# Mouafak-Khaled/Flow-Q-Learning

Hardware: AMD Instinct MI355X
Metric: FQL grad-steps/sec (whole node) over 16-α population, cube-single-v0 (higher is better)
Workload: dtype f32

## Files before the change

flow-q-learning_amd/csrc/kernels.h:

```cpp
#pragma once
#include <hip/hip_runtime.h>
#include <stdint.h>

namespace fq {

struct TRef {
    float* p;
    long long ss;
    long long sy;
};

inline TRef tref(float* p, long long ss, long long sy = 0) { return TRef{p, ss, sy}; }

enum GemmLayout { LAYOUT_FWD = 0, LAYOUT_DX = 1, LAYOUT_DW = 2 };
enum GemmEpi { EPI_STORE = 0, EPI_BIAS = 1, EPI_BIAS_GELU2 = 2, EPI_BIAS_GELU = 3, EPI_ADAM = 4 };

struct GemmArgs {
    TRef A, B, C, C2, bias;
    int M, N, K;
    int lda, ldb, ldc;
    int ny, nz;
    const int* slots;
    unsigned long long* probe;
};
// ... 217 lines not shown
    int nz;
    const int* slots;
};
void launch_input_grad(const InGradArgs& a, hipStream_t s);

struct SampleArgs {
    const float *obs, *act, *rew, *mask, *nobs;
    long long n_rows;
    const float* inj_batch;
    const float* inj_noise;
    const uint64_t* seeds;
    const int* count;
    int step_add;
    unsigned stream_salt;
    int B, D, A;
    TRef os_in;
    TRef bc_in;
    TRef cr_in;
    TRef tg_in;
    TRef eu_in;
    TRef act_t, x0_t, rew_t, mask_t;
    int nz;
    const int* slots;
};
void launch_sample(const SampleArgs& a, hipStream_t s);

struct LossArgs {
    TRef q, qt, rew, mask;
    TRef vpred, act, x0, amet;
    TRef apiraw, aflow, da;
    TRef dq;
    TRef dv;
    TRef dout_os;
    TRef g_cb4, g_bcb4, g_osb4;
    TRef info;
    const float* alpha;
    int B, A, E, da_n;
    int q_min, normq;
    float discount;
    int nz;
    const int* slots;
};
void launch_loss_critic(const LossArgs& a, hipStream_t s);
void launch_loss_bc(const LossArgs& a, hipStream_t s);
void launch_loss_actor(const LossArgs& a, hipStream_t s);

void launch_adam(const AdamArgs& a, hipStream_t s);

struct FinalArgs {
    const float* stats;
    const int* chunk_leaf;
    const int* leaf_first;
    int n_total_chunks, n_leaves;
// ... 52 lines not shown
```

flow-q-learning_amd/csrc/kernels.hip:

```cpp
#include "kernels.h"

#include <hip/hip_runtime.h>
#include <math.h>

#include <type_traits>

#if defined(__HIP_DEVICE_COMPILE__) && !defined(__gfx950__)
#error "fqlpop kernels target gfx950 (MI355X) only: the s_waitcnt immediates use the gfx9 encoding"
#endif


namespace fq {

typedef float f32x16 __attribute__((ext_vector_type(16)));
typedef float f32x4 __attribute__((ext_vector_type(4)));

#define DEV __device__ __forceinline__

DEV float* at(TRef t, int slot, int y = 0) {
    return t.p + (long long)slot * t.ss + (long long)y * t.sy;
}

constexpr float kSqrt2OverPi = 0.7978845608028654f;

// ... 2931 lines not shown
        obs = pb + (long long)b * D;
        actp = pb + (long long)B * D + (long long)b * A;
        rew = pb[(long long)B * (D + A) + b];
        mask = pb[(long long)B * (D + A + 1) + b];
        nobs = pb + (long long)B * (D + A + 2) + (long long)b * D;
    } else {
        const long long idx = (long long)(((unsigned long long)c0[0] * (unsigned long long)a.n_rows) >> 32);
        actp = a.act + idx * A;
        obs = a.obs + idx * D;
        nobs = a.nobs + idx * D;
        rew = a.rew[idx];
        mask = a.mask[idx];
    }
    const float* pn = a.inj_noise ? a.inj_noise + z * (long long)B * (4 * A + 1) : nullptr;
    const float t = pn ? pn[(long long)B * 2 * A + b] : u01(c0[1]);
    auto put = [&](int k, float o, float n) {
        os[k * B3 + b] = n;
        os[k * B3 + B + b] = o;
        os[k * B3 + 2 * B + b] = o;
        bc[k * B2 + b] = o;
        bc[k * B2 + B + b] = o;
        cr[k * B2 + b] = o;
        cr[k * B2 + B + b] = o;
        tg[(long long)k * B + b] = n;
        eu[(long long)k * B + b] = o;
    };
    constexpr int KQ = 8;
    float ov[KQ], nv0[KQ];
#pragma unroll
    for (int q = 0; q < KQ; ++q) {
        const int k = min(p + SP * q, D - 1);
        ov[q] = obs[k];
        nv0[q] = nobs[k];
    }
#pragma unroll
    for (int q = 0; q < KQ; ++q)
        if (p + SP * q < D) put(p + SP * q, ov[q], nv0[q]);
    for (int k = p + SP * KQ; k < D; k += SP) put(k, obs[k], nobs[k]);
    if (p < A) {
        const float av = actp[p];
        cr[(D + p) * B2 + b] = av;
        at(a.act_t, slot)[(long long)p * B + b] = av;
    }
    for (int q = p; 2 * q < 4 * A; q += SP) {
        float nv[2];
        if (pn) {
            for (int h = 0; h < 2; ++h) {
                const int i = 2 * q + h, cat = i / A, j = i % A;
                const long long o = cat == 0 ? (long long)b * A + j
                                  : cat == 1 ? (long long)B * A + b * A + j
                                  : cat == 2 ? (long long)B * (2 * A + 1) + b * A + j
                                             : (long long)B * (3 * A + 1) + b * A + j;
                nv[h] = i < 4 * A ? pn[o] : 0.f;
            }
        } else {
            uint32_t c[4] = {(uint32_t)b, step, a.stream_salt, 1u + (uint32_t)q};
            philox4x32_10(c, (uint32_t)seed, (uint32_t)(seed >> 32));
            const float r = sqrtf(-2.0f * logf(u01_open_closed(c[0])));
            float sv, cv;
            sincosf(6.283185307179586f * u01(c[1]), &sv, &cv);
            nv[0] = r * cv;
            nv[1] = r * sv;
        }
        for (int h = 0; h < 2; ++h) {
            const int i = 2 * q + h;
            if (i >= 4 * A) break;
            const int cat = i / A, j = i % A;
            const long long r = D + j;
            const float v = nv[h];
            if (cat == 0) {
                os[r * B3 + b] = v;
            } else if (cat == 1) {
                at(a.x0_t, slot)[(long long)j * B + b] = v;
                bc[r * B2 + b] = (1.0f - t) * v + t * actp[j];
            } else if (cat == 2) {
                os[r * B3 + B + b] = v;
                bc[r * B2 + B + b] = v;
            } else {
                os[r * B3 + 2 * B + b] = v;
            }
        }
// ... 39 lines not shown
            qs += qv;
            qmx = fmaxf(qmx, qv);
            qmn = fminf(qmn, qv);
            const float g = 2.0f * d * invEB;
            dq[e * a.dq.sy + b] = g;
            if (e < 4) sdq[e] += g;
            qp += q[e * a.q.sy + B + b];
        }
        qp /= (float)E;
        qpi_s += qp;
        qpi_abs += fabsf(qp);
    }
    const float* am = at(a.amet, slot);
    const float* ac = at(a.act, slot);
    float smse = 0.f;
    for (int i = threadIdx.x; i < A * B; i += 256) {
        const float d = am[i] - ac[i];
        smse += d * d;
    }
    float rv[11] = {sq, qs, qmx, qmn, qpi_s, qpi_abs, smse, sdq[0], sdq[1], sdq[2], sdq[3]};
    block_reduce_n<11>(rv, {0, 0, 1, 2, 0, 0, 0, 0, 0, 0, 0}, red);
    sq = rv[0];
    qs = rv[1];
    qmx = rv[2];
    qmn = rv[3];
    qpi_s = rv[4];
    qpi_abs = rv[5];
    smse = rv[6];
    if (threadIdx.x == 0)
        for (int e = 0; e < E && e < 4; ++e) at(a.g_cb4, slot, e)[0] = rv[7 + e];
    const float qmean_pi = qpi_s / (float)B;
    const float lam = a.normq ? 1.0f / (qpi_abs / (float)B) : 1.0f;
    const float gpi = -lam * invEB;
    for (int b = threadIdx.x; b < B; b += 256)
        for (int e = 0; e < E; ++e) dq[e * a.dq.sy + B + b] = gpi;
    if (threadIdx.x == 0) {
        float* info = at(a.info, slot);
        info[0] = sq * invEB;
        info[1] = qs * invEB;
        info[2] = qmx;
        info[3] = qmn;
        info[7] = -lam * qmean_pi;
        info[8] = qmean_pi;
        info[9] = smse / (float)(A * B);
    }
}

__global__ __launch_bounds__(256) void loss_bc_kernel(const LossArgs a) {
    const int z = blockIdx.x, slot = a.slots[z];
    const int B = a.B, A = a.A;
    __shared__ float red[9 * 8];
    const float* vp = at(a.vpred, slot);
    const float* ac = at(a.act, slot);
    const float* x0 = at(a.x0, slot);
    float* dv = at(a.dv, slot);
    const float sc = 2.0f / (float)(A * B);
    float s = 0.f;
    float sdb[8];
#pragma unroll
// ... 406 lines not shown
```

flow-q-learning_amd/csrc/runtime.cpp:

```cpp
#include <hip/hip_runtime.h>

#include <algorithm>
#include <cmath>
#include <cstdio>
#include <cstdlib>
#include <cstring>
#include <functional>
#include <map>
#include <set>
#include <memory>
#include <string>
#include <vector>

#include "../../include/fqlpop.h"
#include "kernels.h"

using namespace fq;

namespace {

thread_local std::string g_err;

struct FqErr {
    int code;
// ... 23 lines not shown

struct EngineOptions {
    int euler_fused = 1;
    int stream_fwd = 1;
    int stream_bwd = 1;
    int fused_adam = 1;
    int serial = 0;
    int dw_tile_critic = 10, dw_tile_actor = 10;
    int adam_nt = 3;
    int split = 1;
    int small_sched = 1;
    int split_blocks = 256;
    int split_sites = 0;
    int hw_queues = 4;
    int em_seq_sweep = 1;
};
EngineOptions g_engine_opts;

constexpr int kStepBranches = 4;
int step_streams(const EngineOptions& eo) {
    return (eo.serial || eo.hw_queues < kStepBranches) ? 1 : kStepBranches;
}

struct EngineOptionRef {
    const char* name;
    int EngineOptions::*field;
    int lo, hi;
};
const EngineOptionRef kEngineOptions[] = {
    {"euler_fused", &EngineOptions::euler_fused, 0, 1}, {"stream_fwd", &EngineOptions::stream_fwd, 0, 1},
    {"stream_bwd", &EngineOptions::stream_bwd, 0, 1},   {"fused_adam", &EngineOptions::fused_adam, 0, 1},
    {"serial", &EngineOptions::serial, 0, 1},
    {"dw_tile_critic", &EngineOptions::dw_tile_critic, 0, 10},
    {"dw_tile_actor", &EngineOptions::dw_tile_actor, 0, 10},
    {"adam_nt", &EngineOptions::adam_nt, 0, 3},
    {"split", &EngineOptions::split, 0, 8},
    {"small_sched", &EngineOptions::small_sched, 0, 1},
    {"hw_queues", &EngineOptions::hw_queues, 1, 1024},
    {"split_sites", &EngineOptions::split_sites, 0, (1 << 24) - 1},
    {"split_blocks", &EngineOptions::split_blocks, 64, 1024},
    {"em_seq_sweep", &EngineOptions::em_seq_sweep, 0, 1},
};

void philox_host(uint32_t c[4], uint32_t k0, uint32_t k1) {
    for (int r = 0; r < 10; ++r) {
        const uint64_t p0 = (uint64_t)0xD2511F53u * c[0], p1 = (uint64_t)0xCD9E8D57u * c[2];
        const uint32_t hi0 = (uint32_t)(p0 >> 32), lo0 = (uint32_t)p0;
        const uint32_t hi1 = (uint32_t)(p1 >> 32), lo1 = (uint32_t)p1;
        const uint32_t n0 = hi1 ^ c[1] ^ k0, n2 = hi0 ^ c[3] ^ k1;
        c[0] = n0; c[1] = lo1; c[2] = n2; c[3] = lo0;
        k0 += 0x9E3779B9u;
        k1 += 0xBB67AE85u;
    }
}

uint64_t sample_key(uint64_t seed, float alpha) {
// ... 142 lines not shown
    long long phase_blocks = 0;
    unsigned long long* ephase_host = nullptr;
    unsigned long long* ephase_dev = nullptr;
    long long ephase_blocks = 0;
    int probe_pairs = 0;
    long long probe_blocks = 0;
    long long probe_nb[2] = {0, 0};
    hipEvent_t probe_done[2] = {nullptr, nullptr};
    hipStream_t probe_stream = nullptr;
    bool probe_pending[2] = {false, false};
    double probe_total_ms = 0.0;
    long long probe_launches = 0;
    long long probe_blocks_seen = 0, probe_blocks_expected = 0;
    double clock_check_event_us = 0.0, clock_check_stamp_us = 0.0;
    std::map<long long, Graphs> graphs;

    float* alloc(long long per_slot) {
        float* p = nullptr;
        HIPCHK(hipMalloc(&p, sizeof(float) * std::max<long long>(1, per_slot * n)));
        HIPCHK(hipMemset(p, 0, sizeof(float) * std::max<long long>(1, per_slot * n)));
        allocs.push_back(p);
        return p;
    }
};

namespace {

void build_leaves(fqlpop* h) {
    struct NetRef { const char* name; int id; const NetLayout* lay; };
    const NetRef order[4] = {{"actor_bc_flow", 2, &h->bc}, {"actor_onestep_flow", 3, &h->os},
// ... 158 lines not shown
    mirror_params(h, slot, h->sM);
    HIPCHK(hipStreamSynchronize(h->sM));
    h->wt_dirty = true;
}

const NetLayout* phase_net(const fqlpop* h) {
    const char* v = diag_env("FQLPOP_PHASE_NET");
    if (v != nullptr && std::strcmp(v, "bc") == 0) return &h->bc;
    if (v != nullptr && std::strcmp(v, "os") == 0) return &h->os;
    return &h->critic;
}

struct Ctx {
    fqlpop* h;
    int nz;
};

TRef pref(fqlpop* h, float* arena, const NetLayout& N, long long off) {
    return tref(arena + N.off + off, h->P, N.ens_size);
}

hipEvent_t next_event(fqlpop* h) {
    if (h->ev_next >= (int)h->ev_pool.size()) throw FqErr{FQLPOP_E_STATE, "event pool exhausted"};
    return h->ev_pool[h->ev_next++];
}

struct TileChoice {
    int tile, variant;
};
TileChoice pick_gemm(int layout, int M, int N, int nyz) {
    const long long t64 = (long long)((M + 63) / 64) * (N / 64) * nyz;
    if (layout == LAYOUT_FWD) {
        if (M % 64 != 0) return {0, 0};
        if (t64 <= 512) return {0, 5};
        if (N % 128 == 0 && N < 768) return {2, 4};
        return {0, 4};
    }
    if (M < 64) return {0, 0};
    if (N % 128 != 0) return {0, 0};
    return {t64 >= 2048 ? 3 : 2, 0};
}

void gemm(int layout, int epi, const GemmArgs& g, hipStream_t s) {
    const TileChoice t = pick_gemm(layout, g.M, g.N, g.ny * g.nz);
    launch_gemm_variant(layout, epi, t.tile, t.variant, g, s);
}

constexpr long long kSmallSchedTiles = 256;
enum { SITE_BCF = 0, SITE_EULER = 1, SITE_OSF = 2, SITE_TGT = 3, SITE_CRF = 4, SITE_CRB = 5, SITE_OSB = 6, SITE_CRB2 = 7,
       SITE_N = 8 };
constexpr long long kSplitMaxClusters = 128;
constexpr long long kSplitMaxClustersSide = 64;
constexpr long long split_cap(int site) {
    return (site == SITE_BCF || site == SITE_TGT || site == SITE_CRF || site == SITE_OSB) ? kSplitMaxClustersSide
                                                                                        : kSplitMaxClusters;
}
constexpr long long kSplitMaxBlocks = 256;

int split_factor_opts(const EngineOptions& o, bool split_ok, int site, long long clusters, bool min4,
// ... 7 lines not shown
    }
    if (!split_ok || opt == 0 || clusters > split_cap(site)) return 1;
    for (int F = std::max(opt >= 2 ? opt : 8, min4 ? 4 : 2); F >= 2; F /= 2) {
        if (min4 && F < 4) break;
        if (clusters * F <= max_blocks) return F;
    }
    return 1;
}
int split_factor(const fqlpop* h, int site, long long clusters, bool min4, long long max_blocks = kSplitMaxBlocks) {
    return split_factor_opts(h->opt, h->split_ok, site, clusters, min4, max_blocks);
}

struct SplitShape {
    int H, L, A, B, E, K0bc, K0os, K0cr;
    bool critic_ln, stream_fwd, stream_bwd, fused_adam, euler_fused, multi_stream;
};
void split_plan(const EngineOptions& o, const SplitShape& d, int nz, int F[SITE_N], bool* small) {
    const bool ok = d.stream_fwd && o.split != 0;
    const int B = d.B, B2 = 2 * B, B3 = 3 * B, T = B / 16;
    auto fwd = [&](int site, int K0, int nout, int M, long long clusters, bool min4) {
        F[site] = d.stream_fwd && split_fwd_supported(d.H, d.L, K0, nout, M)
                      ? split_factor_opts(o, ok, site, clusters, min4, o.split_blocks) : 1;
    };
    fwd(SITE_EULER, d.K0bc, d.A, B, (long long)T * nz, true);
    if (!d.euler_fused) F[SITE_EULER] = 1;
    *small = o.small_sched && d.multi_stream && d.stream_fwd && d.stream_bwd && d.fused_adam &&
             (long long)T * nz <= kSmallSchedTiles;
    fwd(SITE_BCF, d.K0bc, d.A, B2, (long long)(B2 / 16) * nz, false);
    fwd(SITE_OSF, d.K0os, d.A, B3, (long long)(B3 / 16) * nz, false);
    fwd(SITE_TGT, d.K0cr, 1, B, (long long)T * d.E * nz, false);
    fwd(SITE_CRF, d.K0cr, 1, B2, (long long)(B2 / 16) * d.E * nz, false);
    auto bwd = [&](int site, int nout, int M, int Mg, long long clusters, bool min4) {
        F[site] = d.stream_bwd && split_bwd_supported(d.H, d.L, nout, M, Mg)
                      ? split_factor_opts(o, ok, site, clusters, min4, kSplitMaxBlocks) : 1;
    };
    if (*small) {
        bwd(SITE_CRB, 1, B, 0, (long long)T * d.E * nz, d.critic_ln);
        bwd(SITE_CRB2, 1, B, B, (long long)T * d.E * nz, d.critic_ln);
    } else {
        bwd(SITE_CRB, 1, B2, B, (long long)(B2 / 16) * d.E * nz, d.critic_ln);
        F[SITE_CRB2] = 1;
    }
    bwd(SITE_OSB, d.A, B, B, (long long)T * nz, false);
}
SplitShape split_shape(const fqlpop* h) {
    return SplitShape{h->H, h->L, h->A, h->B, h->E, h->bc.in_dim, h->os.in_dim, h->critic.in_dim, h->critic.ln,
                      h->stream_fwd, h->stream_bwd, h->fused_adam, h->euler_fused, h->sX != h->sM};
}
void check_plan(const fqlpop* h, int site, int nz, int F) {
    int plan[SITE_N];
    bool small = false;
    split_plan(h->opt, split_shape(h), nz, plan, &small);
    ARGCHK(plan[site] == F, "split launch differs from the split plan");
}

SplitSync split_prep(fqlpop* h, int site, long long clusters, hipStream_t) {
    fqlpop::SplitSite& st = h->split_site[site];
    ARGCHK(clusters <= st.clusters, "split launch larger than its site");
    return SplitSync{st.xch, st.cnt, st.gen, h->split_err};
}

int bwd_split(const fqlpop* h, int site, const NetLayout& N, int M, int Mg, int nz) {
    if (&N == &h->bc || !split_bwd_supported(N.H, N.L, N.out_dim, M, Mg)) return 1;
    return split_factor(h, site, (long long)(M / 16) * N.E * nz, N.ln, kSplitMaxBlocks);
}

void fwd_hidden(const Ctx& c, hipStream_t s, const NetLayout& N, TRef X, int ldx, int M,
                const std::vector<float*>& U, const std::vector<float*>& G, long long act_sy,
                const std::vector<float*>* MU, const std::vector<float*>* RS, long long st_sy,
                bool store_u, bool euler = false) {
    fqlpop* h = c.h;
    for (int l = 0; l < N.L; ++l) {
        GemmArgs g{};
        g.A = pref(h, h->params, N, N.W[l]);
        g.B = l == 0 ? X : tref(G[l - 1], (long long)N.H * ldx * N.E, act_sy);
        if (N.ln) {
            g.C = tref(U[l], (long long)N.H * ldx * N.E, act_sy);
        } else {
            g.C = tref(store_u ? U[l] : G[l], (long long)N.H * ldx * N.E, act_sy);
            g.C2 = tref(G[l], (long long)N.H * ldx * N.E, act_sy);
        }
        g.bias = pref(h, h->params, N, N.b[l]);
        g.M = N.H; g.N = M; g.K = N.kdim(l);
        g.lda = N.H; g.ldb = ldx; g.ldc = ldx;
        g.ny = N.E; g.nz = c.nz; g.slots = h->slots;
        const int epi = N.ln ? EPI_BIAS : (store_u ? EPI_BIAS_GELU2 : EPI_BIAS_GELU);
        if (euler && l >= 1 && epi == EPI_BIAS_GELU && g.M % 64 == 0 && g.N % 64 == 0) {
            if (h->probe_set >= 0 && h->probe_idx < h->probe_pairs)
                g.probe = h->probe_slots + 2 * h->probe_blocks * ((long long)h->probe_set * h->probe_pairs + h->probe_idx++);
            launch_gemm_euler_hidden(g, s);
        } else {
            gemm(LAYOUT_FWD, epi, g, s);
        }
        if (N.ln) {
            LnArgs a{};
            a.u = tref(U[l], (long long)N.H * ldx * N.E, act_sy);
            a.h = tref(G[l], (long long)N.H * ldx * N.E, act_sy);
            a.mu = tref((*MU)[l], (long long)ldx * N.E, st_sy);
            a.rstd = tref((*RS)[l], (long long)ldx * N.E, st_sy);
            a.gamma = pref(h, h->params, N, N.gam[l]);
            a.beta = pref(h, h->params, N, N.bet[l]);
            a.H = N.H; a.M = M; a.ld = ldx; a.ny = N.E; a.nz = c.nz; a.slots = h->slots;
            launch_ln_gelu_fwd(a, s);
        }
    }
}

// ... 114 lines not shown
    a.L = N.L; a.M = M; a.Mg = Mg; a.nout = N.out_dim;
    a.ny = N.E; a.nz = c.nz; a.slots = h->slots;
    if (ig) {
        ARGCHK(ig->off == Mg && ig->M == M - Mg, "input-grad columns must follow the grad columns");
        ARGCHK(ig->A >= 1 && ig->A <= 8, "fused dQ/da: at most 8 action inputs");
        a.da = ig->da.p; a.da_ss = ig->da.ss; a.da_sy = (long long)ig->A * ig->M;
        a.ld_da = ig->M; a.D0 = ig->D; a.na = ig->A;
    }
    if (h->phase_dev != nullptr && &N == phase_net(h)) {
        ARGCHK((long long)(M / 16) * N.E * c.nz <= h->phase_blocks, "phase probe: too many blocks");
        a.phase = h->phase_dev;
    }
    if (!(skip_mask() & (&N == &h->critic ? 32 : &N == &h->bc ? 64 : 128))) {
        const int site = &N != &h->critic ? SITE_OSB : (s == h->sX && h->sX != h->sM) ? SITE_CRB2 : SITE_CRB;
        const int F = bwd_split(h, site, N, M, Mg, c.nz);
        if (&N != &h->bc) check_plan(h, site, c.nz, F);
        if (F > 1) {
            const long long clusters = (long long)(M / 16) * N.E * c.nz;
            launch_split_bwd(N.ln, F, a, split_prep(h, site, clusters, s), s);
        } else {
            launch_stream_bwd(N.ln, a, s);
        }
    }
    if (Mg == 0) return;
    hipEvent_t ev = nullptr;
    if (sw != s) {
        ev = next_event(h);
        HIPCHK(hipEventRecord(ev, s));
    }
    const int NP = a.NP;
    auto dw_half = [=, &N]() {
// ... 138 lines not shown
    a.x0 = X.p;
    a.x0_ss = X.ss;
    a.ld_x = ldx; a.K0 = N.in_dim; a.L = N.L; a.M = M;
    a.s_ss = s_ss; a.s_sy = s_sy; a.st_ss = st_ss; a.st_sy = st_sy;
    a.ld_s = ldx; a.st_lo = st_lo; a.st_hi = st_hi;
    a.g_hi = g_hi < 0 ? st_hi : g_hi;
    a.head = head;
    a.head.nout = N.out_dim;
    a.ny = N.E; a.nz = c.nz; a.slots = h->slots;
    const int sk = skip_mask();
    const int bit = &N == &h->bc ? 16 : &N == &h->os ? 8 : arena == h->target ? 2 : 4;
    if (sk & bit) return;
    const int site = &N == &h->bc ? SITE_BCF : &N == &h->os ? SITE_OSF : arena == h->target ? SITE_TGT : SITE_CRF;
    const long long clusters = (long long)(M / 16) * N.E * c.nz;
    const int F = split_fwd_supported(N.H, N.L, N.in_dim, N.out_dim, M) ? split_factor(h, site, clusters, false, h->opt.split_blocks) : 1;
    check_plan(h, site, c.nz, F);
    if (F > 1) {
        SplitFwdArgs sa{};
        sa.s = a;
        sa.sync = split_prep(h, site, clusters, s);
        launch_split_fwd(mode, N.ln, false, F, sa, s);
    } else {
        launch_stream_fwd(mode, N.ln, a, s);
    }
}

int euler_split(const fqlpop* h, int nz) {
    const NetLayout& N = h->bc;
    if (!h->euler_fused || !split_fwd_supported(N.H, N.L, N.in_dim, N.out_dim, h->B)) return 1;
    return split_factor(h, SITE_EULER, (long long)(h->B / 16) * nz, true, h->opt.split_blocks);
}
// ... 161 lines not shown
    if (n == 0) return;
    const double us = 0.01 / (double)n, per = us / (double)steps;
    std::fprintf(stderr, "phase probe (split Euler flow, last launch): %lld blocks, %d steps, span %.1f us, block %.1f us, "
                 "start spread %.2f us, prologue %.2f us; blocks per XCC %d %d %d %d %d %d %d %d\n",
                 n, steps, (double)(t1 - t0) * 0.01, blk * us, (double)(tl - t0) * 0.01, pro * us, xcc[0], xcc[1],
                 xcc[2], xcc[3], xcc[4], xcc[5], xcc[6], xcc[7]);
    std::fprintf(stderr, "  layer 0 per step (redundant, no hand-off): %.3f\n", l0 * per);
    for (int l = 1; l < L; ++l)
        std::fprintf(stderr, "  layer %d per step: stage (wait + copy) %.3f | k-loop %.3f | epilogue + publish %.3f\n", l,
                     stg[l] * per, kl[l] * per, ep[l] * per);
    std::fprintf(stderr, "  head per step (wait for the 8 partials + update): %.3f\n", head * per);
}

void flip_params(fqlpop* h);

void enqueue(fqlpop* h, bool train, bool inj_batch, bool inj_noise) {
    const Ctx c{h, h->nz};
    const int B = h->B, D = h->D, A = h->A, H = h->H, E = h->E, L = h->L, S = h->S;
    const int Kc = D + A, Kb = D + A + 1;
    const int B2 = 2 * B, B3 = 3 * B;
    hipStream_t sM = h->sM, sF = h->sF, sB = h->sB, sX = h->sX;
    h->ev_next = 0;
    h->probe_idx = 0;
    h->cr_in = h->cr_in_buf[h->cur];
    if (h->probe_set >= 0 && !h->euler_fused)
        HIPCHK(hipMemsetAsync(h->probe_slots + 2LL * h->probe_blocks * h->probe_set * h->probe_pairs, 0,
                              sizeof(unsigned long long) * 2 * h->probe_blocks * h->probe_pairs, sM));

    auto dep = [&](hipStream_t from, hipStream_t to) {
        if (from == to) return;
        hipEvent_t ev = next_event(h);
        HIPCHK(hipEventRecord(ev, from));
        HIPCHK(hipStreamWaitEvent(to, ev, 0));
    };

    const auto& dset = (!train && h->ds[1].rows > 0) ? h->ds[1] : h->ds[0];
    SampleArgs sa{};
    sa.obs = dset.obs; sa.act = dset.act; sa.rew = dset.rew; sa.mask = dset.mask; sa.nobs = dset.nobs;
    sa.n_rows = dset.rows;
    sa.inj_batch = inj_batch ? h->inj_batch : nullptr;
    sa.inj_noise = inj_noise ? h->inj_noise : nullptr;
    sa.seeds = h->skeys; sa.count = h->count;
    sa.step_add = 0;
    sa.stream_salt = train ? 0x51A7u : 0x5A1Du;
    sa.B = B; sa.D = D; sa.A = A;
    sa.os_in = tref(h->os_in, (long long)Kc * B3);
    sa.bc_in = tref(h->bc_in, (long long)Kb * B2);
    sa.cr_in = tref(h->cr_in, (long long)Kc * B2);
    sa.tg_in = tref(h->tg_in, (long long)Kc * B);
    sa.eu_in = tref(h->eu_in, (long long)Kb * B);
    sa.act_t = tref(h->act_t, (long long)A * B);
    sa.x0_t = tref(h->x0_t, (long long)A * B);
    sa.rew_t = tref(h->rew_t, B);
    sa.mask_t = tref(h->mask_t, B);
    sa.nz = c.nz; sa.slots = h->slots;
    auto os_forward = [&]() {
        const NetLayout& N = h->os;
        HeadArgs ha = head_args(c, N, h->os_g[L - 1], B3, B3, 0);
        ha.o0 = tref(h->apiraw, (long long)A * B); ha.ld0 = B;
        ha.o1 = tref(h->tg_in, (long long)Kc * B); ha.ld1 = B;
        ha.o2 = tref(h->cr_in, (long long)Kc * B2); ha.ld2 = B2;
        ha.o3 = tref(h->amet, (long long)A * B); ha.ld3 = B;
        if (h->stream_fwd) {
            stream_fwd(c, sM, N, h->params, h->P, tref(h->os_in, (long long)Kc * B3), B3, B3, &h->os_u, &h->os_g,
                       nullptr, nullptr, (long long)H * B3, 0, 0, 0, B, 2 * B, HEAD_OS, ha);
        } else {
            fwd_hidden(c, sM, N, tref(h->os_in, (long long)Kc * B3), B3, B3, h->os_u, h->os_g, 0,
                       nullptr, nullptr, 0, true);
            launch_head_fwd(HEAD_OS, ha, sM);
        }
    };
    launch_sample(sa, sM);
    HIPCHK(hipEventRecord(h->ev_sample, sM));
    if (sF != sM) HIPCHK(hipStreamWaitEvent(sF, h->ev_sample, 0));
    if (sB != sM) HIPCHK(hipStreamWaitEvent(sB, h->ev_sample, 0));

    float* info = train ? h->info : h->vinfo;
    LossArgs la{};
    la.q = tref(h->q, (long long)E * B2, B2);
    la.qt = tref(h->qt, (long long)E * B, B);
    la.rew = tref(h->rew_t, B);
    la.mask = tref(h->mask_t, B);
    la.vpred = tref(h->vpred, (long long)A * B);
// ... 2 lines not shown
    la.amet = tref(h->amet, (long long)A * B);
    la.apiraw = tref(h->apiraw, (long long)A * B);
    la.aflow = tref(h->aflow, (long long)A * B);
    la.da = tref(h->da, (long long)E * A * B, (long long)A * B);
    la.da_n = h->stream_bwd ? E : 1;
    la.dq = tref(h->dq, (long long)E * B2, B2);
    la.dv = tref(h->dv, (long long)A * B);
    la.dout_os = tref(h->dout_os, (long long)A * B);
    la.g_cb4 = pref(h, h->grads, h->critic, h->critic.b[L]);
    la.g_bcb4 = pref(h, h->grads, h->bc, h->bc.b[L]);
    la.g_osb4 = pref(h, h->grads, h->os, h->os.b[L]);
    la.info = tref(info, FQLPOP_INFO_STRIDE);
    la.alpha = h->alpha;
    la.B = B; la.A = A; la.E = E;
    la.q_min = h->cfg.q_agg_min; la.normq = h->cfg.normalize_q_loss;
    la.discount = h->cfg.discount;
    la.nz = c.nz; la.slots = h->slots;

    {
        const NetLayout& N = h->bc;
        HeadArgs ha = head_args(c, N, h->bc_g[L - 1], B2, B2, 0);
        ha.o0 = tref(h->vpred, (long long)A * B); ha.ld0 = B;
        ha.o1 = tref(h->bc_in, (long long)Kb * B2); ha.ld1 = B2;
        ha.o2 = tref(h->eu_in, (long long)Kb * B); ha.ld2 = B;
        ha.t_next = (float)(1.0 / (double)S);
        if (h->stream_fwd) {
            stream_fwd(c, sF, N, h->params, h->P, tref(h->bc_in, (long long)Kb * B2), B2, B2, &h->bc_u, &h->bc_g,
                       nullptr, nullptr, (long long)H * B2, 0, 0, 0, 0, B, HEAD_BC_FUSED, ha);
        } else {
            fwd_hidden(c, sF, N, tref(h->bc_in, (long long)Kb * B2), B2, B2, h->bc_u, h->bc_g, 0,
// ... 34 lines not shown
        if (!h->fused_adam) {
            adam_net(c, sB, 1);
            if (h->stream_bwd) transpose_nets(h, sB, 2, false, h->params_nx, h->paramsT_nx);
        }
    }
    HIPCHK(hipEventRecord(h->ev_bdone, sB));

    os_forward();
    const NetLayout& NC = h->critic;
    const long long sy2 = (long long)H * B2, sy1 = (long long)H * B;
    const bool small = h->opt.small_sched && h->sX != h->sM && h->stream_fwd && h->stream_bwd && h->fused_adam &&
                       (long long)(h->B / 16) * c.nz <= kSmallSchedTiles;
    {
        int plan[SITE_N];
        bool plan_small = false;
        split_plan(h->opt, split_shape(h), c.nz, plan, &plan_small);
        ARGCHK(plan_small == small && plan[SITE_EULER] == euler_split(h, c.nz), "step differs from the split plan");
    }
    hipStream_t sT = small ? h->sX : sM;
    dep(sM, sT);
    if (h->stream_fwd) {
        HeadArgs ht{};
        ht.B = B; ht.D = D; ht.steps_f = (float)S;
        ht.o0 = tref(h->qt, (long long)E * B, B); ht.ld0 = B;
        stream_fwd(c, sT, NC, h->target, h->PT, tref(h->tg_in, (long long)Kc * B), B, B, nullptr, nullptr, nullptr,
                   nullptr, 0, 0, 0, 0, 0, 0, HEAD_STORE, ht);
    } else {
        const NetLayout& N = NC;
        for (int l = 0; l < L; ++l) {
            GemmArgs g{};
            g.A = tref(h->target + N.W[l], h->PT, N.ens_size);
// ... 109 lines not shown
        launch_finalize(fa, sM);
    } else if (sB != sM) {
        HIPCHK(hipStreamWaitEvent(sM, h->ev_bdone, 0));
    }
    HIPCHK(hipGetLastError());
}

void flip_params(fqlpop* h) {
    h->cur ^= 1;
    h->params = h->params_buf[h->cur];
    h->params_nx = h->params_buf[h->cur ^ 1];
    h->paramsT = h->paramsT_buf[h->cur];
    h->paramsT_nx = h->paramsT_buf[h->cur ^ 1];
}

Graphs& graph_for(fqlpop* h, bool train, bool inj_batch, bool inj_noise, bool recapture);

void run(fqlpop* h, bool train, bool inj_batch, bool inj_noise) {
    if (h->nz == 0) return;
    if (h->stream_bwd && h->wt_dirty) {
        transpose_nets(h, h->sM, 7, true, h->params, h->paramsT);
        transpose_nets(h, h->sM, 7, true, h->params, h->paramsT_nx);
        h->wt_dirty = false;
    }
    if (!h->cfg.use_graph) {
        enqueue(h, train, inj_batch, inj_noise);
        if (train) flip_params(h);
        return;
    }
    Graphs& gr = graph_for(h, train, inj_batch, inj_noise, false);
    HIPCHK(hipGraphLaunch(gr.exec, h->sM));
    if (train) flip_params(h);
}

Graphs& graph_for(fqlpop* h, bool train, bool inj_batch, bool inj_noise, bool recapture) {
    const long long key = ((train ? 4 : 0) + (inj_batch ? 2 : 0) + (inj_noise ? 1 : 0)) + 8LL * h->nz +
                          (1LL << 32) * (h->probe_set + 1) + (1LL << 36) * h->cur;
    Graphs& gr = h->graphs[key];
    if (recapture || gr.exec == nullptr || gr.nz != h->nz) {
        if (gr.exec) HIPCHK(hipGraphExecDestroy(gr.exec));
        gr.exec = nullptr;
        hipGraph_t graph;
        {
            std::vector<hipStream_t> ss;
            for (hipStream_t s : {h->sM, h->sF, h->sB, h->sX})
                if (std::find(ss.begin(), ss.end(), s) == ss.end()) ss.push_back(s);
            if ((int)ss.size() > 1 && (int)ss.size() > h->opt.hw_queues)
                throw FqErr{FQLPOP_E_STATE, "step graph would have " + std::to_string(ss.size()) +
                                                " parallel branches on " + std::to_string(h->opt.hw_queues) +
                                                " hardware queues (hipGraphLaunch is unsafe then)"};
        }
        HIPCHK(hipStreamBeginCapture(h->sM, hipStreamCaptureModeRelaxed));
        try {
            enqueue(h, train, inj_batch, inj_noise);
        } catch (...) {
            (void)hipStreamEndCapture(h->sM, &graph);
            throw;
        }
        HIPCHK(hipStreamEndCapture(h->sM, &graph));
        HIPCHK(hipGraphInstantiate(&gr.exec, graph, nullptr, nullptr, 0));
        HIPCHK(hipGraphUpload(gr.exec, h->sM));
        HIPCHK(hipGraphDestroy(graph));
        gr.nz = h->nz;
    }
    return gr;
}

double probe_launch_us(const unsigned long long* v, long long blocks) {
    unsigned long long lo = ~0ULL, hi = 0;
    for (long long b = 0; b < blocks; ++b) {
        if (v[2 * b] == 0 || v[2 * b + 1] == 0) continue;
        lo = std::min(lo, v[2 * b]);
        hi = std::max(hi, v[2 * b + 1]);
    }
    return hi > lo ? (double)(hi - lo) * 0.01 : -1.0;
}

void probe_consume(fqlpop* h, int set) {
    HIPCHK(hipEventSynchronize(h->probe_done[set]));
    const long long per = 2 * h->probe_blocks;
// ... 471 lines not shown
            if (!h->active[i]) mirror_params(h, i, h->sM);
        HIPCHK(hipStreamSynchronize(h->sM));
        h->wt_dirty = true;
    });
}

int fqlpop_step(fqlpop_t* h, int n_steps) {
    return guard([&] {
        ARGCHK(h, "null handle");
        ARGCHK(n_steps >= 0, "n_steps must be >= 0");
        if (split_error_pending(h)) sync_all_streams(h);
        check_split_error(h, -1, true);
        if (h->ds[0].rows == 0) throw FqErr{FQLPOP_E_STATE, "no training dataset set (fqlpop_set_dataset)"};
        HIPCHK(hipSetDevice(h->device));
        for (int i = 0; i < n_steps; ++i) {
            if (h->probe) {
                const int set = (int)(h->probe_step & 1);
                if (h->probe_pending[set]) probe_consume(h, set);
                h->probe_set = set;
                h->probe_nb[set] = euler_blocks(h, h->nz);
                run(h, true, false, false);
                h->probe_set = -1;
                HIPCHK(hipEventRecord(h->probe_done[set], h->sM));
                h->probe_pending[set] = true;
                ++h->probe_step;
            } else {
                run(h, true, false, false);
            }
        }
    });
}

static void stage_injected(fqlpop* h, const float* batch, const float* noise) {
    if (batch)
        HIPCHK(hipMemcpyAsync(h->inj_batch, batch, sizeof(float) * h->inj_bs * h->nz, hipMemcpyHostToDevice, h->sM));
    if (noise)
        HIPCHK(hipMemcpyAsync(h->inj_noise, noise, sizeof(float) * h->inj_ns * h->nz, hipMemcpyHostToDevice, h->sM));
}

int fqlpop_step_injected(fqlpop_t* h, const float* batch, const float* noise) {
    return guard([&] {
        ARGCHK(h && batch, "null argument");
// ... 229 lines not shown
    return guard([&] {
        ARGCHK(h, "null handle");
        HIPCHK(hipSetDevice(h->device));
        sync_all_streams(h);
        if (absorb_split_error(h)) throw FqErr{FQLPOP_E_STATE, kSplitFailMsg};
    });
}

int fqlpop_debug_fail_split(fqlpop_t* h) {
    return guard([&] {
        ARGCHK(h, "null handle");
        HIPCHK(hipSetDevice(h->device));
        if (!h->split_err_host) throw FqErr{FQLPOP_E_STATE, "this population runs no split launch"};
        sync_all_streams(h);
        __atomic_store_n(h->split_err_host, 1u, __ATOMIC_RELEASE);
    });
}

int fqlpop_time_dominant_kernel(fqlpop_t* h, int iters, double* avg_us, double* flops) {
    return guard([&] {
        ARGCHK(h && avg_us && flops && iters > 0, "bad argument");
        HIPCHK(hipSetDevice(h->device));
        HIPCHK(hipDeviceSynchronize());
        const NetLayout& N = h->bc;
        const int B = h->B, H = h->H;
        EulerArgs ea = euler_args(h, h->nz);
        GemmArgs g{};
        g.A = pref(h, h->params, N, N.W[1]);
        g.B = tref(h->eu_g[0], (long long)H * B);
        g.C = tref(h->eu_g[1], (long long)H * B);
// ... 238 lines not shown
```

flow-q-learning_amd/fqlpop/_lib.py:

```python
from __future__ import annotations

import ctypes
import os

try:
    import torch
except Exception:
    torch = None

_HERE = os.path.dirname(os.path.abspath(__file__))
LIB_PATH = os.path.join(_HERE, "libfqlpop.so")

INFO_STRIDE = 16
TRAIN_INFO_KEYS = (
    "critic/critic_loss", "critic/q_mean", "critic/q_max", "critic/q_min",
    "actor/actor_loss", "actor/bc_flow_loss", "actor/distill_loss",
    "actor/q_loss", "actor/q", "actor/mse",
    "grad/max", "grad/min", "grad/norm",
)
VAL_INFO_KEYS = TRAIN_INFO_KEYS[:10]
STATE_PARAMS, STATE_ADAM_M, STATE_ADAM_V = 0, 1, 2


class FqlpopError(RuntimeError):
# ... 66 lines not shown
                                             ctypes.c_uint64, _F]),
    "fqlpop_state_size": (ctypes.c_int, [_P, ctypes.POINTER(ctypes.c_int64)]),
    "fqlpop_get_state": (ctypes.c_int, [_P, ctypes.c_int, ctypes.c_int, _F, ctypes.c_int64]),
    "fqlpop_set_state": (ctypes.c_int, [_P, ctypes.c_int, ctypes.c_int, _F, ctypes.c_int64]),
    "fqlpop_get_count": (ctypes.c_int, [_P, ctypes.c_int, ctypes.POINTER(ctypes.c_int32)]),
    "fqlpop_set_count": (ctypes.c_int, [_P, ctypes.c_int, ctypes.c_int32]),
    "fqlpop_set_member": (ctypes.c_int, [_P, ctypes.c_int, ctypes.c_float, ctypes.c_uint64,
                                         ctypes.c_int]),
    "fqlpop_num_leaves": (ctypes.c_int, [_P, ctypes.POINTER(ctypes.c_int)]),
    "fqlpop_leaf_info": (ctypes.c_int, [_P, ctypes.c_int, ctypes.c_char_p, ctypes.c_int,
                                        ctypes.POINTER(ctypes.c_int64),
                                        ctypes.POINTER(ctypes.c_int),
                                        ctypes.POINTER(ctypes.c_int64)]),
    "fqlpop_sync": (ctypes.c_int, [_P]),
    "fqlpop_debug_fail_split": (ctypes.c_int, [_P]),
    "fqlpop_time_dominant_kernel": (ctypes.c_int, [_P, ctypes.c_int,
                                                   ctypes.POINTER(ctypes.c_double),
                                                   ctypes.POINTER(ctypes.c_double)]),
    "fqlpop_flops_per_member_step": (ctypes.c_double, [ctypes.POINTER(Config)]),
    "fqlpop_set_probe": (ctypes.c_int, [_P, ctypes.c_int]),
    "fqlpop_dominant_kernel_info": (ctypes.c_int, [_P, ctypes.c_char_p, ctypes.c_int,
                                                   ctypes.POINTER(ctypes.c_double),
                                                   ctypes.POINTER(ctypes.c_double)]),
    "fqlpop_read_probe": (ctypes.c_int, [_P, ctypes.POINTER(ctypes.c_double), ctypes.POINTER(ctypes.c_int64),
                                         ctypes.POINTER(ctypes.c_double)]),
    "fqlpop_envmodel_param_count": (ctypes.c_int, [ctypes.POINTER(EnvModelConfig), ctypes.POINTER(ctypes.c_int64),
                                                   ctypes.POINTER(ctypes.c_int64)]),
    "fqlpop_set_env_model": (ctypes.c_int, [_P, ctypes.POINTER(EnvModelConfig), _F, ctypes.c_int64, _F,
                                            ctypes.c_int64]),
    "fqlpop_rollout": (ctypes.c_int, [_P, _F, ctypes.c_int, ctypes.c_int, ctypes.c_uint64, _F, _F, _F]),
# ... 80 lines not shown
```

flow-q-learning_amd/fqlpop/population.py:

```python
from __future__ import annotations

import ctypes
from dataclasses import dataclass

import numpy as np

from fqlpop import _lib
from fqlpop._lib import (INFO_STRIDE, STATE_ADAM_M, STATE_ADAM_V, STATE_PARAMS,
                         TRAIN_INFO_KEYS, VAL_INFO_KEYS, check, fptr)


@dataclass
class PopulationConfig:
    obs_dim: int = 28
    action_dim: int = 5
    hidden_dims: tuple = (512, 512, 512, 512)
    batch_size: int = 256
    num_qs: int = 2
    layer_norm: bool = True
    actor_layer_norm: bool = False
    flow_steps: int = 10
    q_agg: str = "mean"
    normalize_q_loss: bool = False
    discount: float = 0.99
# ... 305 lines not shown
        self.seeds[member] = seed

    def state_dict(self, member: int) -> dict:
        return {"params": self.get_params(member),
                "opt_state": {"count": self.get_count(member),
                              "mu": self.flat_to_tree(self.get_flat(member, STATE_ADAM_M)),
                              "nu": self.flat_to_tree(self.get_flat(member, STATE_ADAM_V))},
                "alpha": float(self.alphas[member]), "seed": int(self.seeds[member])}

    def load_state_dict(self, member: int, sd: dict):
        self.set_params(member, sd["params"])
        self.set_flat(member, self.tree_to_flat(sd["opt_state"]["mu"]), STATE_ADAM_M)
        self.set_flat(member, self.tree_to_flat(sd["opt_state"]["nu"]), STATE_ADAM_V)
        self.set_count(member, int(sd["opt_state"]["count"]))

    def set_probe(self, enable: bool = True):
        check(self.lib.fqlpop_set_probe(self._h, int(bool(enable))))

    def read_probe(self):
        tot = ctypes.c_double()
        n = ctypes.c_int64()
        cc = (ctypes.c_double * 2)()
        check(self.lib.fqlpop_read_probe(self._h, ctypes.byref(tot), ctypes.byref(n), cc))
        mean = tot.value / n.value if n.value else float("nan")
        return mean, int(n.value), (float(cc[0]), float(cc[1]))

    def probe_coverage(self):
        seen, exp = ctypes.c_int64(), ctypes.c_int64()
        check(self.lib.fqlpop_probe_coverage(self._h, ctypes.byref(seen), ctypes.byref(exp)))
        return int(seen.value), int(exp.value)
# ... 17 lines not shown
```

include/fqlpop.h:

```cpp
#ifndef FQLPOP_H
#define FQLPOP_H

#include <stddef.h>
#include <stdint.h>

#ifdef __cplusplus
extern "C" {
#endif

#define FQLPOP_OK 0
#define FQLPOP_E_ARG (-1)
#define FQLPOP_E_HIP (-2)
#define FQLPOP_E_STATE (-3)
#define FQLPOP_E_UNSUPPORTED (-4)

#define FQLPOP_INFO_STRIDE 16
enum {
    FQLPOP_INFO_CRITIC_LOSS = 0, FQLPOP_INFO_Q_MEAN, FQLPOP_INFO_Q_MAX, FQLPOP_INFO_Q_MIN,
    FQLPOP_INFO_ACTOR_LOSS, FQLPOP_INFO_BC_FLOW_LOSS, FQLPOP_INFO_DISTILL_LOSS,
    FQLPOP_INFO_Q_LOSS, FQLPOP_INFO_Q, FQLPOP_INFO_MSE,
    FQLPOP_INFO_GRAD_MAX, FQLPOP_INFO_GRAD_MIN, FQLPOP_INFO_GRAD_NORM
};

enum { FQLPOP_STATE_PARAMS = 0, FQLPOP_STATE_ADAM_M = 1, FQLPOP_STATE_ADAM_V = 2 };
// ... 53 lines not shown

int fqlpop_get_state(fqlpop_t* h, int member, int which, float* flat, int64_t n);
int fqlpop_set_state(fqlpop_t* h, int member, int which, const float* flat, int64_t n);

int fqlpop_get_count(fqlpop_t* h, int member, int32_t* count);
int fqlpop_set_count(fqlpop_t* h, int member, int32_t count);

int fqlpop_set_member(fqlpop_t* h, int member, float alpha, uint64_t seed, int reinit);

int fqlpop_num_leaves(fqlpop_t* h, int* n);
int fqlpop_leaf_info(fqlpop_t* h, int i, char* name, int name_cap, int64_t* offset,
                     int* ndim, int64_t* shape3);

int fqlpop_sync(fqlpop_t* h);
int fqlpop_debug_fail_split(fqlpop_t* h);

int fqlpop_time_dominant_kernel(fqlpop_t* h, int iters, double* avg_us, double* flops);

int fqlpop_set_probe(fqlpop_t* h, int enable);
int fqlpop_dominant_kernel_info(fqlpop_t* h, char* name, int name_cap, double* flops, double* bytes);
int fqlpop_read_probe(fqlpop_t* h, double* total_us, int64_t* launches, double* clock_check);
int fqlpop_probe_coverage(fqlpop_t* h, int64_t* blocks_seen, int64_t* blocks_expected);

typedef struct fqlpop_envmodel_config {
    int obs_dim, action_dim;
    int sp_num_hidden;
    int sp_hidden[7];
    int tp_num_hidden;
    int tp_hidden[7];
} fqlpop_envmodel_config;
// ... 57 lines not shown
```

Measured before the change: 8388.

## Skip metric-only work on quiet train steps via separate graph variant

Adds a quiet train-step mode that runs on every step except the last of a batch. On those steps the one-step policy forward covers 2B rows instead of 3B, the metric noise is neither generated nor written, and the action-MSE reduction is skipped. Two CUDA/HIP graphs (reporting and quiet) are captured and cached per key. This removes the work that only feeds logged metrics from most steps, at the cost of doubling graph captures and leaving some info fields stale on quiet steps.

```diff
diff --git a/flow-q-learning_amd/csrc/kernels.h b/flow-q-learning_amd/csrc/kernels.h
--- a/flow-q-learning_amd/csrc/kernels.h
+++ b/flow-q-learning_amd/csrc/kernels.h
@@ -255,6 +255,7 @@
     int step_add;
     unsigned stream_salt;
     int B, D, A;
+    int metric;
     TRef os_in;
     TRef bc_in;
     TRef cr_in;
@@ -278,6 +279,7 @@
     const float* alpha;
     int B, A, E, da_n;
     int q_min, normq;
+    int metric;
     float discount;
     int nz;
     const int* slots;
diff --git a/flow-q-learning_amd/csrc/kernels.hip b/flow-q-learning_amd/csrc/kernels.hip
--- a/flow-q-learning_amd/csrc/kernels.hip
+++ b/flow-q-learning_amd/csrc/kernels.hip
@@ -2969,10 +2969,11 @@
     }
     const float* pn = a.inj_noise ? a.inj_noise + z * (long long)B * (4 * A + 1) : nullptr;
     const float t = pn ? pn[(long long)B * 2 * A + b] : u01(c0[1]);
+    const bool metric = a.metric != 0;
     auto put = [&](int k, float o, float n) {
         os[k * B3 + b] = n;
         os[k * B3 + B + b] = o;
-        os[k * B3 + 2 * B + b] = o;
+        if (metric) os[k * B3 + 2 * B + b] = o;
         bc[k * B2 + b] = o;
         bc[k * B2 + B + b] = o;
         cr[k * B2 + b] = o;
@@ -2997,7 +2998,8 @@
         cr[(D + p) * B2 + b] = av;
         at(a.act_t, slot)[(long long)p * B + b] = av;
     }
-    for (int q = p; 2 * q < 4 * A; q += SP) {
+    const int n_noise = metric ? 4 * A : 3 * A;
+    for (int q = p; 2 * q < n_noise; q += SP) {
         float nv[2];
         if (pn) {
             for (int h = 0; h < 2; ++h) {
@@ -3019,7 +3021,7 @@
         }
         for (int h = 0; h < 2; ++h) {
             const int i = 2 * q + h;
-            if (i >= 4 * A) break;
+            if (i >= n_noise) break;
             const int cat = i / A, j = i % A;
             const long long r = D + j;
             const float v = nv[h];
@@ -3089,10 +3091,11 @@
     const float* am = at(a.amet, slot);
     const float* ac = at(a.act, slot);
     float smse = 0.f;
-    for (int i = threadIdx.x; i < A * B; i += 256) {
-        const float d = am[i] - ac[i];
-        smse += d * d;
-    }
+    if (a.metric)
+        for (int i = threadIdx.x; i < A * B; i += 256) {
+            const float d = am[i] - ac[i];
+            smse += d * d;
+        }
     float rv[11] = {sq, qs, qmx, qmn, qpi_s, qpi_abs, smse, sdq[0], sdq[1], sdq[2], sdq[3]};
     block_reduce_n<11>(rv, {0, 0, 1, 2, 0, 0, 0, 0, 0, 0, 0}, red);
     sq = rv[0];
@@ -3117,7 +3120,7 @@
         info[3] = qmn;
         info[7] = -lam * qmean_pi;
         info[8] = qmean_pi;
-        info[9] = smse / (float)(A * B);
+        if (a.metric) info[9] = smse / (float)(A * B);
     }
 }
 
diff --git a/flow-q-learning_amd/csrc/runtime.cpp b/flow-q-learning_amd/csrc/runtime.cpp
--- a/flow-q-learning_amd/csrc/runtime.cpp
+++ b/flow-q-learning_amd/csrc/runtime.cpp
@@ -61,6 +61,7 @@
     int split_sites = 0;
     int hw_queues = 4;
     int em_seq_sweep = 1;
+    int metrics_every_step = 0;
 };
 EngineOptions g_engine_opts;
 
@@ -87,6 +88,7 @@
     {"split_sites", &EngineOptions::split_sites, 0, (1 << 24) - 1},
     {"split_blocks", &EngineOptions::split_blocks, 64, 1024},
     {"em_seq_sweep", &EngineOptions::em_seq_sweep, 0, 1},
+    {"metrics_every_step", &EngineOptions::metrics_every_step, 0, 1},
 };
 
 void philox_host(uint32_t c[4], uint32_t k0, uint32_t k1) {
@@ -259,6 +261,7 @@
     long long probe_blocks_seen = 0, probe_blocks_expected = 0;
     double clock_check_event_us = 0.0, clock_check_stamp_us = 0.0;
     std::map<long long, Graphs> graphs;
+    long long graph_captures = 0;
 
     float* alloc(long long per_slot) {
         float* p = nullptr;
@@ -447,6 +450,7 @@
 struct Ctx {
     fqlpop* h;
     int nz;
+    bool report;
 };
 
 TRef pref(fqlpop* h, float* arena, const NetLayout& N, long long off) {
@@ -474,8 +478,8 @@
     return {t64 >= 2048 ? 3 : 2, 0};
 }
 
-void gemm(int layout, int epi, const GemmArgs& g, hipStream_t s) {
-    const TileChoice t = pick_gemm(layout, g.M, g.N, g.ny * g.nz);
+void gemm(int layout, int epi, const GemmArgs& g, hipStream_t s, int pick_N = 0) {
+    const TileChoice t = pick_gemm(layout, g.M, pick_N > 0 ? pick_N : g.N, g.ny * g.nz);
     launch_gemm_variant(layout, epi, t.tile, t.variant, g, s);
 }
 
@@ -513,10 +517,11 @@
 struct SplitShape {
     int H, L, A, B, E, K0bc, K0os, K0cr;
     bool critic_ln, stream_fwd, stream_bwd, fused_adam, euler_fused, multi_stream;
+    bool report = true;
 };
 void split_plan(const EngineOptions& o, const SplitShape& d, int nz, int F[SITE_N], bool* small) {
     const bool ok = d.stream_fwd && o.split != 0;
-    const int B = d.B, B2 = 2 * B, B3 = 3 * B, T = B / 16;
+    const int B = d.B, B2 = 2 * B, Mos = d.report ? 3 * B : 2 * B, T = B / 16;
     auto fwd = [&](int site, int K0, int nout, int M, long long clusters, bool min4) {
         F[site] = d.stream_fwd && split_fwd_supported(d.H, d.L, K0, nout, M)
                       ? split_factor_opts(o, ok, site, clusters, min4, o.split_blocks) : 1;
@@ -526,7 +531,7 @@
     *small = o.small_sched && d.multi_stream && d.stream_fwd && d.stream_bwd && d.fused_adam &&
              (long long)T * nz <= kSmallSchedTiles;
     fwd(SITE_BCF, d.K0bc, d.A, B2, (long long)(B2 / 16) * nz, false);
-    fwd(SITE_OSF, d.K0os, d.A, B3, (long long)(B3 / 16) * nz, false);
+    fwd(SITE_OSF, d.K0os, d.A, Mos, (long long)(Mos / 16) * nz, false);
     fwd(SITE_TGT, d.K0cr, 1, B, (long long)T * d.E * nz, false);
     fwd(SITE_CRF, d.K0cr, 1, B2, (long long)(B2 / 16) * d.E * nz, false);
     auto bwd = [&](int site, int nout, int M, int Mg, long long clusters, bool min4) {
@@ -542,14 +547,14 @@
     }
     bwd(SITE_OSB, d.A, B, B, (long long)T * nz, false);
 }
-SplitShape split_shape(const fqlpop* h) {
+SplitShape split_shape(const fqlpop* h, bool report) {
     return SplitShape{h->H, h->L, h->A, h->B, h->E, h->bc.in_dim, h->os.in_dim, h->critic.in_dim, h->critic.ln,
-                      h->stream_fwd, h->stream_bwd, h->fused_adam, h->euler_fused, h->sX != h->sM};
-}
-void check_plan(const fqlpop* h, int site, int nz, int F) {
+                      h->stream_fwd, h->stream_bwd, h->fused_adam, h->euler_fused, h->sX != h->sM, report};
+}
+void check_plan(const fqlpop* h, int site, int nz, int F, bool report) {
     int plan[SITE_N];
     bool small = false;
-    split_plan(h->opt, split_shape(h), nz, plan, &small);
+    split_plan(h->opt, split_shape(h, report), nz, plan, &small);
     ARGCHK(plan[site] == F, "split launch differs from the split plan");
 }
 
@@ -567,7 +572,7 @@
 void fwd_hidden(const Ctx& c, hipStream_t s, const NetLayout& N, TRef X, int ldx, int M,
                 const std::vector<float*>& U, const std::vector<float*>& G, long long act_sy,
                 const std::vector<float*>* MU, const std::vector<float*>* RS, long long st_sy,
-                bool store_u, bool euler = false) {
+                bool store_u, bool euler = false, int pick_cols = 0) {
     fqlpop* h = c.h;
     for (int l = 0; l < N.L; ++l) {
         GemmArgs g{};
@@ -589,7 +594,7 @@
                 g.probe = h->probe_slots + 2 * h->probe_blocks * ((long long)h->probe_set * h->probe_pairs + h->probe_idx++);
             launch_gemm_euler_hidden(g, s);
         } else {
-            gemm(LAYOUT_FWD, epi, g, s);
+            gemm(LAYOUT_FWD, epi, g, s, pick_cols);
         }
         if (N.ln) {
             LnArgs a{};
@@ -734,7 +739,7 @@
     if (!(skip_mask() & (&N == &h->critic ? 32 : &N == &h->bc ? 64 : 128))) {
         const int site = &N != &h->critic ? SITE_OSB : (s == h->sX && h->sX != h->sM) ? SITE_CRB2 : SITE_CRB;
         const int F = bwd_split(h, site, N, M, Mg, c.nz);
-        if (&N != &h->bc) check_plan(h, site, c.nz, F);
+        if (&N != &h->bc) check_plan(h, site, c.nz, F, c.report);
         if (F > 1) {
             const long long clusters = (long long)(M / 16) * N.E * c.nz;
             launch_split_bwd(N.ln, F, a, split_prep(h, site, clusters, s), s);
@@ -903,7 +908,7 @@
     const int site = &N == &h->bc ? SITE_BCF : &N == &h->os ? SITE_OSF : arena == h->target ? SITE_TGT : SITE_CRF;
     const long long clusters = (long long)(M / 16) * N.E * c.nz;
     const int F = split_fwd_supported(N.H, N.L, N.in_dim, N.out_dim, M) ? split_factor(h, site, clusters, false, h->opt.split_blocks) : 1;
-    check_plan(h, site, c.nz, F);
+    check_plan(h, site, c.nz, F, c.report);
     if (F > 1) {
         SplitFwdArgs sa{};
         sa.s = a;
@@ -1095,8 +1100,9 @@
 
 void flip_params(fqlpop* h);
 
-void enqueue(fqlpop* h, bool train, bool inj_batch, bool inj_noise) {
-    const Ctx c{h, h->nz};
+void enqueue(fqlpop* h, bool train, bool inj_batch, bool inj_noise, bool report) {
+    ARGCHK(report || train, "only a train step can be quiet");
+    const Ctx c{h, h->nz, report};
     const int B = h->B, D = h->D, A = h->A, H = h->H, E = h->E, L = h->L, S = h->S;
     const int Kc = D + A, Kb = D + A + 1;
     const int B2 = 2 * B, B3 = 3 * B;
@@ -1125,6 +1131,7 @@
     sa.step_add = 0;
     sa.stream_salt = train ? 0x51A7u : 0x5A1Du;
     sa.B = B; sa.D = D; sa.A = A;
+    sa.metric = report ? 1 : 0;
     sa.os_in = tref(h->os_in, (long long)Kc * B3);
     sa.bc_in = tref(h->bc_in, (long long)Kb * B2);
     sa.cr_in = tref(h->cr_in, (long long)Kc * B2);
@@ -1137,17 +1144,18 @@
     sa.nz = c.nz; sa.slots = h->slots;
     auto os_forward = [&]() {
         const NetLayout& N = h->os;
-        HeadArgs ha = head_args(c, N, h->os_g[L - 1], B3, B3, 0);
+        const int Mos = report ? B3 : B2;
+        HeadArgs ha = head_args(c, N, h->os_g[L - 1], B3, Mos, 0);
         ha.o0 = tref(h->apiraw, (long long)A * B); ha.ld0 = B;
         ha.o1 = tref(h->tg_in, (long long)Kc * B); ha.ld1 = B;
         ha.o2 = tref(h->cr_in, (long long)Kc * B2); ha.ld2 = B2;
         ha.o3 = tref(h->amet, (long long)A * B); ha.ld3 = B;
         if (h->stream_fwd) {
-            stream_fwd(c, sM, N, h->params, h->P, tref(h->os_in, (long long)Kc * B3), B3, B3, &h->os_u, &h->os_g,
+            stream_fwd(c, sM, N, h->params, h->P, tref(h->os_in, (long long)Kc * B3), B3, Mos, &h->os_u, &h->os_g,
                        nullptr, nullptr, (long long)H * B3, 0, 0, 0, B, 2 * B, HEAD_OS, ha);
         } else {
-            fwd_hidden(c, sM, N, tref(h->os_in, (long long)Kc * B3), B3, B3, h->os_u, h->os_g, 0,
-                       nullptr, nullptr, 0, true);
+            fwd_hidden(c, sM, N, tref(h->os_in, (long long)Kc * B3), B3, Mos, h->os_u, h->os_g, 0,
+                       nullptr, nullptr, 0, true, false, B3);
             launch_head_fwd(HEAD_OS, ha, sM);
         }
     };
@@ -1180,6 +1188,7 @@
     la.alpha = h->alpha;
     la.B = B; la.A = A; la.E = E;
     la.q_min = h->cfg.q_agg_min; la.normq = h->cfg.normalize_q_loss;
+    la.metric = report ? 1 : 0;
     la.discount = h->cfg.discount;
     la.nz = c.nz; la.slots = h->slots;
 
@@ -1244,7 +1253,7 @@
     {
         int plan[SITE_N];
         bool plan_small = false;
-        split_plan(h->opt, split_shape(h), c.nz, plan, &plan_small);
+        split_plan(h->opt, split_shape(h, report), c.nz, plan, &plan_small);
         ARGCHK(plan_small == small && plan[SITE_EULER] == euler_split(h, c.nz), "step differs from the split plan");
     }
     hipStream_t sT = small ? h->sX : sM;
@@ -1384,9 +1393,9 @@
     h->paramsT_nx = h->paramsT_buf[h->cur ^ 1];
 }
 
-Graphs& graph_for(fqlpop* h, bool train, bool inj_batch, bool inj_noise, bool recapture);
-
-void run(fqlpop* h, bool train, bool inj_batch, bool inj_noise) {
+Graphs& graph_for(fqlpop* h, bool train, bool inj_batch, bool inj_noise, bool report);
+
+void run(fqlpop* h, bool train, bool inj_batch, bool inj_noise, bool report = true) {
     if (h->nz == 0) return;
     if (h->stream_bwd && h->wt_dirty) {
         transpose_nets(h, h->sM, 7, true, h->params, h->paramsT);
@@ -1394,20 +1403,29 @@
         h->wt_dirty = false;
     }
     if (!h->cfg.use_graph) {
-        enqueue(h, train, inj_batch, inj_noise);
+        enqueue(h, train, inj_batch, inj_noise, report);
         if (train) flip_params(h);
         return;
     }
-    Graphs& gr = graph_for(h, train, inj_batch, inj_noise, false);
+    Graphs& gr = graph_for(h, train, inj_batch, inj_noise, report);
     HIPCHK(hipGraphLaunch(gr.exec, h->sM));
     if (train) flip_params(h);
 }
 
-Graphs& graph_for(fqlpop* h, bool train, bool inj_batch, bool inj_noise, bool recapture) {
-    const long long key = ((train ? 4 : 0) + (inj_batch ? 2 : 0) + (inj_noise ? 1 : 0)) + 8LL * h->nz +
-                          (1LL << 32) * (h->probe_set + 1) + (1LL << 36) * h->cur;
-    Graphs& gr = h->graphs[key];
-    if (recapture || gr.exec == nullptr || gr.nz != h->nz) {
+Graphs& graph_for(fqlpop* h, bool train, bool inj_batch, bool inj_noise, bool report) {
+    const long long base = ((train ? 4 : 0) + (inj_batch ? 2 : 0) + (inj_noise ? 1 : 0)) + 8LL * h->nz +
+                           (1LL << 32) * (h->probe_set + 1) + (1LL << 36) * h->cur;
+    auto key = [&](bool rep) { return base + (1LL << 37) * (rep ? 1 : 0); };
+    const bool both = train && !inj_batch && !inj_noise;
+    ARGCHK(report || both, "only a device-sampled train step can be quiet");
+    auto missing = [&](bool rep) {
+        const auto it = h->graphs.find(key(rep));
+        return it == h->graphs.end() || it->second.exec == nullptr || it->second.nz != h->nz;
+    };
+    for (int v = 0; v < (both ? 2 : 1); ++v) {
+        const bool rep = both ? v == 0 : report;
+        if (!missing(rep)) continue;
+        Graphs& gr = h->graphs[key(rep)];
         if (gr.exec) HIPCHK(hipGraphExecDestroy(gr.exec));
         gr.exec = nullptr;
         hipGraph_t graph;
@@ -1422,7 +1440,7 @@
         }
         HIPCHK(hipStreamBeginCapture(h->sM, hipStreamCaptureModeRelaxed));
         try {
-            enqueue(h, train, inj_batch, inj_noise);
+            enqueue(h, train, inj_batch, inj_noise, rep);
         } catch (...) {
             (void)hipStreamEndCapture(h->sM, &graph);
             throw;
@@ -1432,8 +1450,9 @@
         HIPCHK(hipGraphUpload(gr.exec, h->sM));
         HIPCHK(hipGraphDestroy(graph));
         gr.nz = h->nz;
-    }
-    return gr;
+        ++h->graph_captures;
+    }
+    return h->graphs[key(report)];
 }
 
 double probe_launch_us(const unsigned long long* v, long long blocks) {
@@ -1935,18 +1954,19 @@
         if (h->ds[0].rows == 0) throw FqErr{FQLPOP_E_STATE, "no training dataset set (fqlpop_set_dataset)"};
         HIPCHK(hipSetDevice(h->device));
         for (int i = 0; i < n_steps; ++i) {
+            const bool report = i == n_steps - 1 || h->opt.metrics_every_step != 0 || (i & 0xFFFFF) == 0xFFFFF;
             if (h->probe) {
                 const int set = (int)(h->probe_step & 1);
                 if (h->probe_pending[set]) probe_consume(h, set);
                 h->probe_set = set;
                 h->probe_nb[set] = euler_blocks(h, h->nz);
-                run(h, true, false, false);
+                run(h, true, false, false, report);
                 h->probe_set = -1;
                 HIPCHK(hipEventRecord(h->probe_done[set], h->sM));
                 h->probe_pending[set] = true;
                 ++h->probe_step;
             } else {
-                run(h, true, false, false);
+                run(h, true, false, false, report);
             }
         }
     });
@@ -2206,6 +2226,13 @@
         if (!h->split_err_host) throw FqErr{FQLPOP_E_STATE, "this population runs no split launch"};
         sync_all_streams(h);
         __atomic_store_n(h->split_err_host, 1u, __ATOMIC_RELEASE);
+    });
+}
+
+int fqlpop_debug_graph_captures(fqlpop_t* h, long long* n) {
+    return guard([&] {
+        ARGCHK(h && n, "null argument");
+        *n = h->graph_captures;
     });
 }
 
diff --git a/flow-q-learning_amd/fqlpop/_lib.py b/flow-q-learning_amd/fqlpop/_lib.py
--- a/flow-q-learning_amd/fqlpop/_lib.py
+++ b/flow-q-learning_amd/fqlpop/_lib.py
@@ -104,6 +104,7 @@
                                         ctypes.POINTER(ctypes.c_int64)]),
     "fqlpop_sync": (ctypes.c_int, [_P]),
     "fqlpop_debug_fail_split": (ctypes.c_int, [_P]),
+    "fqlpop_debug_graph_captures": (ctypes.c_int, [_P, ctypes.POINTER(ctypes.c_longlong)]),
     "fqlpop_time_dominant_kernel": (ctypes.c_int, [_P, ctypes.c_int,
                                                    ctypes.POINTER(ctypes.c_double),
                                                    ctypes.POINTER(ctypes.c_double)]),
diff --git a/flow-q-learning_amd/fqlpop/population.py b/flow-q-learning_amd/fqlpop/population.py
--- a/flow-q-learning_amd/fqlpop/population.py
+++ b/flow-q-learning_amd/fqlpop/population.py
@@ -343,6 +343,11 @@
         self.set_flat(member, self.tree_to_flat(sd["opt_state"]["nu"]), STATE_ADAM_V)
         self.set_count(member, int(sd["opt_state"]["count"]))
 
+    def graph_captures(self) -> int:
+        n = ctypes.c_longlong()
+        check(self.lib.fqlpop_debug_graph_captures(self._h, ctypes.byref(n)))
+        return int(n.value)
+
     def set_probe(self, enable: bool = True):
         check(self.lib.fqlpop_set_probe(self._h, int(bool(enable))))
 
diff --git a/include/fqlpop.h b/include/fqlpop.h
--- a/include/fqlpop.h
+++ b/include/fqlpop.h
@@ -91,6 +91,7 @@
 
 int fqlpop_sync(fqlpop_t* h);
 int fqlpop_debug_fail_split(fqlpop_t* h);
+int fqlpop_debug_graph_captures(fqlpop_t* h, long long* n);
 
 int fqlpop_time_dominant_kernel(fqlpop_t* h, int iters, double* avg_us, double* flops);
 
```

New measurement: 8463, median of 6. No clear change (+0.9%).
